# dan64/vs-deoldify

Hardware: AMD Instinct MI355X
Metric: colorized frames/sec/GPU @1080p (DeOldify stable rf=35); CIEDE2000 vs ref (higher is better)
Workload: dtype f16

## Files before the change

vsdeoldify_amd/csrc/conv_igemm.hip:

```cpp
#include "conv_common.h"

__device__ __forceinline__ int swz(int row) { return (4 - ((row >> 2) & 3)) & 3; }

template <int BM, int BN, int WM, int WN, bool PRECISE = false>
__global__ void __launch_bounds__(256, (BN > 256 ? 1 : 2)) conv_igemm_kernel(const ConvArgs p) {
    constexpr int FM = BM / WM / 16;
    constexpr int FN = BN / WN / 16;
    constexpr int A_IT = BM * 4 / 256;
    constexpr int B_IT = (BN * 4 + 255) / 256;
    constexpr int STAGE = (BM + BN) * 32;
    static_assert(BM % 64 == 0, "BM");
    __shared__ __attribute__((aligned(16))) half_t smem[2 * STAGE];

    const int tid = threadIdx.x;
    const int lane = tid & 63, wave = tid >> 6;
    const int wm = wave / WN, wn = wave % WN;
    const int lr = lane & 15, lg = lane >> 4;

    const int nwg = gridDim.x;
    int pid;
    {
        const int orig = blockIdx.x, xcd = orig & 7, q = nwg >> 3, r = nwg & 7;
        pid = (xcd < r ? xcd * (q + 1) : r * (q + 1) + (xcd - r) * q) + (orig >> 3);
    }
// ... 120 lines not shown
    const int64_t blocks128 = (int64_t)((a.M + 127) / 128) * ((a.Npad + 127) / 128);
    if (a.Npad <= 64) return a.M >= 128 * 256 ? CFG_128x64 : CFG_64x64;
    if (blocks128 >= 512) return CFG_128x128;
    const int64_t blocks64x128 = (int64_t)((a.M + 63) / 64) * ((a.Npad + 127) / 128);
    if (blocks64x128 >= 512 || a.Npad % 128 == 0) return CFG_64x128;
    return CFG_64x64;
}

bool conv_pipe_supported(const ConvArgs& a, int extra);

static int pick_pipe(const ConvArgs& a) {
    if (a.flags & HAVC_F_OUT_RGB8) return 0;
    const int extra = (a.Npad % 256 == 16) ? 1 : 0;
    if (!conv_pipe_supported(a, extra)) return 0;
    if (a.flags & HAVC_F_PS_BLUR) return extra ? 0 : 60;
    if (a.flags & HAVC_F_FUSE_RGB8) return 61;
    if (a.flags & HAVC_F_FUSE_PROJ) return (extra || a.Npad % 256) ? 0 : 60;
    if (a.Npad >= 256 && (a.Npad % 256 == 0 || extra)) {
        const int64_t blocks = (int64_t)((a.M + 255) / 256) * ((a.Npad - 16 * extra) / 256);
        if (blocks >= 160) return 60 + extra;
    }
    if (a.Npad % 128 == 0) {
        const int64_t blocks128 = (int64_t)((a.M + 127) / 128) * (a.Npad / 128);
        return blocks128 >= 200 ? 70 : 72;
    }
    return 0;
}

const char* conv_config_name(const ConvArgs& a) {
    switch (pick_pipe(a)) {
        case 60: return "pipe256x256";
        case 61: return "pipe256x272";
        case 70: return "pipe128x128";
        case 72: return "pipe64x128";
    }
    static const char* names[] = {"128x128", "128x64", "64x64", "128x272", "128x304", "128x16", "64x128"};
    return names[pick_config(a)];
}

int launch_conv(const ConvArgs& a, hipStream_t s) {
    if (a.splitk > 1) {
        int cfg = a.cfg;
        if (!conv_splitk_cfg_ok(cfg)) cfg = a.Npad % 256 == 0 ? 71 : (a.Npad % 128 == 0 ? 72 : (a.Npad <= 64 ? 92 : 72));
        if (!conv_pipe_supported(a, 0)) return (int)hipErrorInvalidValue;
        return launch_conv_pipe(a, cfg, s);
    }
    if ((a.flags & HAVC_F_FUSE_PROJ) && a.cfg != 0 && a.cfg != 60) return (int)hipErrorInvalidValue;
// ... 20 lines not shown
```

vsdeoldify_amd/csrc/conv_igemm_pipe.hip:

```cpp
#include "conv_common.h"
#include <atomic>
#include <cstdio>
#include <cstdlib>
#include <type_traits>

#include "conv_pipe_kernel.inc"

template <int EXTRA, int ABL = 0>
__global__ void __launch_bounds__(512) conv_halo_kernel(const ConvArgs p) {
    constexpr int WM = 2, WN = 4, FM = 8, NW = 8, BM = 256, BN = 256, B_IT = BN / 8 / NW, NS = 16;
    constexpr int HB = 46 * 1024, WB = (BN + 16 * EXTRA) * 128, H_IT = 6, HP = 144;
    extern __shared__ __attribute__((aligned(16))) char smem[];
    char* const Wbase = smem + 2 * HB;

    const int tid = threadIdx.x;
    const int lane = tid & 63;
    const int wave = __builtin_amdgcn_readfirstlane(tid >> 6);
    const int wm = wave / WN, wn = wave % WN;
    const int lr = lane & 15, lg = lane >> 4;

    const int nwg = gridDim.x;
    int pid;
    {
        const int orig = blockIdx.x, xcd = orig & 7, q = nwg >> 3, r = nwg & 7;
        pid = (xcd < r ? xcd * (q + 1) : r * (q + 1) + (xcd - r) * q) + (orig >> 3);
    }
    const int NT = (p.Npad - 16 * EXTRA + BN - 1) / BN;
    const int tile = pid / NT;
    const int m0 = tile * BM;
    const int n0 = (pid % NT) * BN;
    const bool has_extra = EXTRA && (n0 + BN + 16 == p.Npad);
    const int HoWo = p.Ho * p.Wo;
    const int tt = p.tiles_y * p.tiles_x;
    const int tb = tile / tt, trem = tile - tb * tt, ty = trem / p.tiles_x, tx = trem - ty * p.tiles_x;

    const __amdgpu_buffer_rsrc_t rx = __builtin_amdgcn_make_buffer_rsrc(const_cast<half_t*>(p.x), 0, p.x_bytes, 0x00020000);
    const __amdgpu_buffer_rsrc_t rw = __builtin_amdgcn_make_buffer_rsrc(const_cast<half_t*>(p.w), 0, p.w_bytes, 0x00020000);

    const int r8 = lane >> 3;
    const int c = (lane & 7) ^ ((((wave & 1) << 2) + (r8 >> 1)) & 7);
    unsigned b_voff[B_IT];
#pragma unroll
    for (int it = 0; it < B_IT; ++it) {
        const int n = n0 + (wave + it * NW) * 8 + r8;
        b_voff[it] = n < p.Npad ? (unsigned)((n * p.Kc + c) * 16) : OOB;
    }
    const unsigned x_voff = (unsigned)(((n0 + BN + (wave & 1) * 8 + r8) * p.Kc + c) * 16);
    const bool extra_wave = has_extra && wave >= 6;

    unsigned h_voff[H_IT];
#pragma unroll
    for (int it = 0; it < H_IT; ++it) {
        const int piece = wave + it * NW;
        const int sl = piece * 64 + lane;
        const int row = sl / 9, col = sl - row * 9;
        const int hy = row / 18, hx = row - hy * 18;
        const int iy = ty * 16 - 1 + hy, ix = tx * 16 - 1 + hx;
        const bool ok = piece < 46 && row < 324 && col < 8 && (unsigned)iy < (unsigned)p.Hi && (unsigned)ix < (unsigned)p.Wi;
        const int chunk = (col & 4) | ((col & 1) << 1) | ((col >> 1) & 1);
        const unsigned off = (unsigned)((((int64_t)(tb * p.Hi + iy) * p.Wi + ix) * p.x_cpitch + p.x_coff) * 2) + (unsigned)chunk * 16u;
        h_voff[it] = ok ? (off | (col == 0 ? 1u : 0u)) : OOB;
    }
    const int G = p.C8a >> 3;
    const int KT = p.Kc >> 3;
    const bool has_rem = KT > 9 * G;

    const int fsw = (lr >> 1) & 7;
    const int b_l0 = (wn * 64 + lr) * 128 + ((lg ^ fsw) << 4), b_l1 = b_l0 ^ 64;
    const int x_l0 = (BN + lr) * 128 + ((lg ^ fsw) << 4), x_l1 = x_l0 ^ 64;
    const int lp = lr < 4 ? 2 * lr : (lr < 12 ? 2 * (lr - 4) + 1 : 2 * (lr - 8));
    const int a_row = (wm * 8 * 18 + lp) * HP;
    int a_cur = a_row + (((lg & 1) << 1) | (lg >> 1)) * 16, a_nxt = a_cur + HB;
    auto tap_off = [](int t) { return ((t / 3) * 18 + (t % 3)) * HP; };
    const int rem_buf = (G & 1) * HB;
    const int a_rem0 = rem_buf + a_row + tap_off(lg), a_rem1 = rem_buf + a_row + tap_off(4 + lg), a_rem8 = rem_buf + a_row + tap_off(8);

    float4v acc[FN][FM];
    float4v accx[2];
#pragma unroll
    for (int ni = 0; ni < FN; ++ni)
#pragma unroll
        for (int mi = 0; mi < FM; ++mi) acc[ni][mi] = float4v{0.f, 0.f, 0.f, 0.f};
    accx[0] = accx[1] = float4v{0.f, 0.f, 0.f, 0.f};

    auto w_piece = [&](int q, char* wbuf, int kstage, bool live = true) {
        dma16(rw, wbuf + (wave + q * NW) * 1024, (ABL == 6 || !live) ? OOB : b_voff[q], (unsigned)kstage * 128u);
    };
    auto h_piece = [&](int it, int hoff, int group, bool rem, bool live = true) {
        const unsigned v = h_voff[it];
        const unsigned vr = (v & 1u) ? (v & ~1u) : OOB;
        const unsigned vo = (ABL == 6 || !live) ? OOB : (rem ? vr : (v & ~1u));
        dma16(rx, smem + hoff + (wave + it * NW) * 1024, vo, (unsigned)group * 128u);
    };

#pragma unroll
    for (int it = 0; it < H_IT; ++it) if (wave + it * NW < 46) h_piece(it, 0, 0, G == 0);
#pragma unroll
    for (int q = 0; q < B_IT; ++q) w_piece(q, Wbase, 0);
    if (EXTRA && extra_wave) dma16(rw, Wbase + BN * 128 + (wave & 1) * 1024, x_voff, 0);
    if (KT > 1) {
#pragma unroll
        for (int q = 0; q < B_IT; ++q) w_piece(q, Wbase + WB, 1);
        if (EXTRA && extra_wave) dma16(rw, Wbase + WB + BN * 128 + (wave & 1) * 1024, x_voff, 128u);
    }
    asm volatile("s_waitcnt vmcnt(0)" ::: "memory");
    __builtin_amdgcn_s_barrier();

    half8 bf[2][FN];
    half8 xb[2];
    half8 af[4];
#pragma unroll
    for (int ni = 0; ni < FN; ++ni) bf[0][ni] = *reinterpret_cast<const half8*>(Wbase + b_l0 + ni * 2048);
    if (EXTRA) xb[0] = *reinterpret_cast<const half8*>(Wbase + x_l0);
    {
        const int a0 = G > 0 ? a_cur : a_rem0;
        af[0] = *reinterpret_cast<const half8*>(smem + a0);
        af[1] = *reinterpret_cast<const half8*>(smem + a0 + 18 * HP);
    }
    int h_cur_off = 0;

    auto stage = [&](int kt, int group, auto t_tag, int a_next) {
        constexpr int T = decltype(t_tag)::value;
        constexpr bool DMA_ON = ABL != 1;
        const char* wcur = Wbase + (kt & 1) * WB;
        char* wnxt = Wbase + ((kt & 1) ^ 1) * WB;
        const bool more2 = kt + 2 < KT;
#pragma unroll
        for (int s = 0; s < NS; ++s) {
            const int ks = s / FM, mi = s % FM;
            if (s + 2 < NS) {
                const int s2 = s + 2, k2 = s2 / FM, m2 = s2 % FM;
                int addr;
                if (T < 9) addr = a_cur + tap_off(T) + m2 * 18 * HP + k2 * 64;
                else if (T == 9) addr = (k2 ? a_rem1 : a_rem0) + m2 * 18 * HP;
                else addr = a_rem8 + m2 * 18 * HP;
                af[s2 % 4] = *reinterpret_cast<const half8*>(smem + addr);
            }
            if (s == NS - 3) {
                asm volatile("s_waitcnt vmcnt(0) lgkmcnt(0)" ::: "memory");
                __builtin_amdgcn_s_barrier();
            }
            if (s >= NS - 2) {
                const int j = s - (NS - 2);
                af[(s + 2) % 4] = *reinterpret_cast<const half8*>(smem + a_next + j * 18 * HP);
#pragma unroll
                for (int ni = 2 * j; ni < 2 * j + 2; ++ni) bf[0][ni] = *reinterpret_cast<const half8*>(wnxt + b_l0 + ni * 2048);
                if (EXTRA && j == 1) xb[0] = *reinterpret_cast<const half8*>(wnxt + x_l0);
            }
            if (ks == 0 && mi >= FM - FN)
                bf[1][mi - (FM - FN)] = *reinterpret_cast<const half8*>(wcur + b_l1 + (mi - (FM - FN)) * 2048);
            if (EXTRA && s == 3) xb[1] = *reinterpret_cast<const half8*>(wcur + x_l1);
            if (DMA_ON) {
                if (s >= NS - 3) {
                    char* wc = const_cast<char*>(wcur);
                    if (s == NS - 3) w_piece(0, wc, kt + 2, more2);
                    if (s == NS - 2) { w_piece(1, wc, kt + 2, more2); w_piece(2, wc, kt + 2, more2); }
                    if (s == NS - 1) {
                        w_piece(3, wc, kt + 2, more2);
                        if (EXTRA) { if (extra_wave) dma16(rw, wc + BN * 128 + (wave & 1) * 1024, more2 ? x_voff : OOB, (unsigned)(kt + 2) * 128u); }
                    }
                }
                if (T < H_IT && s == 6) {
                    if (T < H_IT - 1 || wave + T * NW < 46) h_piece(T, h_cur_off ^ HB, group + 1, group + 1 >= G, group + 1 < G || has_rem);
                }
            }
            const half8 a = af[s % 4];
#pragma unroll
            for (int ni = 0; ni < FN; ++ni) {
                if (ABL == 4) asm volatile("" ::"v"(bf[ks][ni]), "v"(a));
                else acc[ni][mi] = __builtin_amdgcn_mfma_f32_16x16x32_f16(bf[ks][ni], a, acc[ni][mi], 0, 0, 0);
            }
            if (EXTRA && has_extra) {
                if (wn == (mi >> 1)) accx[mi & 1] = __builtin_amdgcn_mfma_f32_16x16x32_f16(xb[ks], a, accx[mi & 1], 0, 0, 0);
            }
            __builtin_amdgcn_sched_barrier(0);
        }
    };
    int kt = 0;
    for (int g = 0; g < G; ++g) {
        stage(kt++, g, std::integral_constant<int, 0>{}, a_cur + tap_off(1));
        stage(kt++, g, std::integral_constant<int, 1>{}, a_cur + tap_off(2));
        stage(kt++, g, std::integral_constant<int, 2>{}, a_cur + tap_off(3));
        stage(kt++, g, std::integral_constant<int, 3>{}, a_cur + tap_off(4));
        stage(kt++, g, std::integral_constant<int, 4>{}, a_cur + tap_off(5));
        stage(kt++, g, std::integral_constant<int, 5>{}, a_cur + tap_off(6));
        stage(kt++, g, std::integral_constant<int, 6>{}, a_cur + tap_off(7));
        stage(kt++, g, std::integral_constant<int, 7>{}, a_cur + tap_off(8));
        stage(kt++, g, std::integral_constant<int, 8>{}, g + 1 < G ? a_nxt : a_rem0);
        const int t = a_cur; a_cur = a_nxt; a_nxt = t;
        h_cur_off ^= HB;
    }
    if (has_rem) {
        stage(kt++, G, std::integral_constant<int, 9>{}, a_rem8);
        stage(kt++, G, std::integral_constant<int, 10>{}, a_rem8);
    }

    auto gm = [&](int local_row) -> int {
        const int y = ty * 16 + (local_row >> 4), x = tx * 16 + (local_row & 15);
        return (y < p.Ho && x < p.Wo) ? (tb * p.Ho + y) * p.Wo + x : 0x7fffffff;
    };
#define PF(mi) (mi)
#define HAVC_STAMP(i) do { } while (0)
    const int eflags = p.flags;
    constexpr bool UNIT_STEP = false;
    auto opix = [&](int m) -> int64_t { return (int64_t)m; };
#include "conv_pipe_epilogue.inc"
#undef PF
#undef HAVC_STAMP
}

template <int EXTRA, int ABL = 0>
static int launch_halo(const ConvArgs& a0, hipStream_t s) {
    ConvArgs a = a0;
    if ((a.Kc & 7) || a.x_bytes == 0 || a.x_bytes >= OOB || a.w_bytes >= OOB || a.kh != 3 || a.kw != 3 || a.stride != 1 || a.pad != 1 ||
        a.pad_w != 1 || a.dil != 1 || a.oss != 1 || a.Hi != a.Ho || a.Wi != a.Wo)
        return (int)hipErrorInvalidValue;
    const int frames = a.M / (a.Ho * a.Wo);
    a.tiles_y = (a.Ho + 15) / 16;
    a.tiles_x = (a.Wo + 15) / 16;
    const int MT = frames * a.tiles_y * a.tiles_x, NT = (a.Npad - 16 * EXTRA + 255) / 256;
    a.M = MT * 256;
    constexpr int LDS = 2 * 46 * 1024 + 2 * (256 + 16 * EXTRA) * 128;
    static_assert(LDS <= 160 * 1024, "LDS budget");
    ensure_lds_optin<conv_halo_kernel<EXTRA, ABL>>(LDS);
    hipLaunchKernelGGL((conv_halo_kernel<EXTRA, ABL>), dim3(MT * NT), dim3(512), LDS, s, a);
    return (int)hipGetLastError();
}

__global__ void splitk_reduce_kernel(const ConvArgs p) {
    const int n4 = p.Npad >> 2, HoWo = p.Ho * p.Wo;
    const int64_t total = (int64_t)p.M * n4;
    for (int64_t i = blockIdx.x * (int64_t)blockDim.x + threadIdx.x; i < total; i += (int64_t)gridDim.x * blockDim.x) {
        const int m = (int)(i / n4), n = (int)(i - (int64_t)m * n4) * 4;
        float4v acc = *reinterpret_cast<const float4v*>(p.ws + (int64_t)m * p.Npad + n);
        for (int sp = 1; sp < p.splitk; ++sp) {
            const float4v t = *reinterpret_cast<const float4v*>(p.ws + ((int64_t)sp * p.M + m) * p.Npad + n);
            acc[0] += t[0]; acc[1] += t[1]; acc[2] += t[2]; acc[3] += t[3];
        }
        epilogue_frag(p, acc, m, n, HoWo);
    }
}

// ... 18 lines not shown
    const int64_t work = (int64_t)a.M * (a.Npad >> 2);
    const int64_t gb = (work + 255) / 256;
    hipLaunchKernelGGL(splitk_reduce_kernel, dim3((unsigned)(gb > 8192 ? 8192 : gb)), dim3(256), 0, s, a);
    return (int)hipGetLastError();
}

void preload_conv_pipe() {
#define PL(WM, WN, FM, EX, ABL) ensure_lds_optin<conv_pipe_kernel<WM, WN, FM, EX, ABL>>(Geo<WM, WN, FM, EX>::LDS_BYTES)
    PL(2, 4, 8, 0, 0); PL(2, 4, 8, 1, 0); PL(2, 2, 4, 0, 0); PL(1, 4, 8, 0, 0); PL(1, 2, 4, 0, 0);
    PL(1, 4, 6, 0, 0); PL(1, 4, 4, 0, 0); PL(2, 2, 6, 0, 0); PL(1, 2, 6, 0, 0); PL(2, 4, 4, 0, 0); PL(2, 4, 6, 0, 0); PL(4, 2, 4, 0, 0);
    PL(4, 1, 4, 0, 0); PL(2, 1, 4, 0, 0);
    PL(2, 4, 8, 0, 30); PL(2, 4, 8, 1, 30); PL(2, 2, 4, 0, 30); PL(1, 4, 8, 0, 30); PL(1, 2, 4, 0, 30); PL(2, 4, 4, 0, 30); PL(4, 2, 4, 0, 30);
    PL(4, 1, 4, 0, 30); PL(2, 1, 4, 0, 30);
#undef PL
    preload_conv_pipe_ef();
    ensure_lds_optin<conv_halo_kernel<0, 0>>(2 * 46 * 1024 + 2 * 256 * 128);
    ensure_lds_optin<conv_halo_kernel<1, 0>>(2 * 46 * 1024 + 2 * 272 * 128);
    (void)hipGetLastError();
}

bool conv_splitk_cfg_ok(int cfg) {
    switch (cfg) { case 60: case 70: case 71: case 72: case 90: case 91: case 92: case 93: case 95: case 96: case 97: case 98: case 99: return true; }
    return false;
}

bool conv_pipe_supported(const ConvArgs& a, int extra) {
    return !(a.Kc & 7) && a.ktab && a.x_bytes != 0 && a.x_bytes < OOB && a.w_bytes < OOB && (!extra || a.Npad == 272);
}

int launch_conv_pipe(const ConvArgs& a, int cfg, hipStream_t s) {
    if (a.flags & HAVC_F_PRECISE) {
        switch (cfg) {
            case 60: return launch_pipe<2, 4, 8, 0, 30>(a, s);
            case 61: return launch_pipe<2, 4, 8, 1, 30>(a, s);
            case 70: return launch_pipe<2, 2, 4, 0, 30>(a, s);
            case 71: return launch_pipe<1, 4, 8, 0, 30>(a, s);
            case 72: return launch_pipe<1, 2, 4, 0, 30>(a, s);
            case 96: return launch_pipe<2, 4, 4, 0, 30>(a, s);
            case 98: return launch_pipe<4, 2, 4, 0, 30>(a, s);
            case 99: return launch_pipe<4, 1, 4, 0, 30>(a, s);
            case 92: return launch_pipe<2, 1, 4, 0, 30>(a, s);
        }
        return (int)hipErrorInvalidValue;
    }
    {
        const int r = launch_conv_pipe_ef(a, cfg, s);
        if (r != -1) return r;
        static const bool trace = getenv("HAVC_EPI_TRACE") != nullptr;
        if (trace) {
            static std::atomic<uint64_t> seen[64];
            const uint64_t key = ((uint64_t)cfg << 32) | (uint32_t)(a.flags & 0xffff) | ((uint64_t)(a.splitk > 1) << 48) | ((uint64_t)(a.oss != 1) << 49) | ((uint64_t)(!a.bias) << 50);
            for (auto& e : seen) {
                uint64_t cur = e.load();
                if (cur == key) break;
                if (cur == 0 && e.compare_exchange_strong(cur, key)) {
                    fprintf(stderr, "havc: run-time-flag conv kernel: cfg %d flags 0x%x splitk %d out_step %d bias %d (M %d, N %d, K %d)\n", cfg, a.flags & 0xffff, a.splitk, a.oss,
                            a.bias != nullptr, a.M, a.Npad, a.Kc * 8);
                    break;
                }
                if (cur == key) break;
            }
// ... 8 lines not shown
        case 103: return launch_pipe<2, 4, 8, 1, 22>(a, s);
        case 62: return launch_pipe<2, 4, 8, 0, 1>(a, s);
        case 64: return launch_pipe<2, 4, 8, 0, 4>(a, s);
        case 69: return launch_pipe<2, 4, 8, 0, 9>(a, s);
        case 73: return launch_pipe<2, 4, 8, 0, 10>(a, s);
        case 65: return launch_pipe<2, 4, 8, 0, 5>(a, s);
        case 162: return launch_pipe<2, 4, 8, 0, 40, 0>(a, s);
        case 163: return launch_pipe<2, 4, 8, 0, 40, HAVC_F_GELU>(a, s);
        case 164: return launch_pipe<2, 4, 8, 1, 40, HAVC_F_RELU_PRE>(a, s);
        case 68: return launch_pipe<2, 4, 8, 0, 12>(a, s);
        case 78: return launch_pipe<2, 4, 8, 0, 14>(a, s);
        case 66: return launch_pipe<2, 4, 8, 0, 11>(a, s);
        case 67: return launch_pipe<2, 4, 8, 0, 13>(a, s);
        case 80: return launch_halo<0>(a, s);
        case 81: return launch_halo<1>(a, s);
        case 82: return launch_halo<0, 1>(a, s);
        case 84: return launch_halo<0, 4>(a, s);
        case 85: return launch_halo<0, 5>(a, s);
        case 86: return launch_halo<0, 6>(a, s);
        case 70: return launch_pipe<2, 2, 4, 0>(a, s);
        case 71: return launch_pipe<1, 4, 8, 0>(a, s);
        case 72: return launch_pipe<1, 2, 4, 0>(a, s);
        case 90: return launch_pipe<1, 4, 6, 0>(a, s);
        case 91: return launch_pipe<1, 4, 4, 0>(a, s);
        case 93: return launch_pipe<2, 2, 6, 0>(a, s);
        case 95: return launch_pipe<1, 2, 6, 0>(a, s);
        case 96: return launch_pipe<2, 4, 4, 0>(a, s);
        case 97: return launch_pipe<2, 4, 6, 0>(a, s);
        case 98: return launch_pipe<4, 2, 4, 0>(a, s);
        case 99: return launch_pipe<4, 1, 4, 0>(a, s);
// ... 9 lines not shown
```

vsdeoldify_amd/csrc/kernels.h:

```cpp
#pragma once
#include <hip/hip_runtime.h>
#include <stdint.h>

typedef _Float16 half_t;

struct ConvArgs {
    const half_t* x;
    const half_t* w;
    const float* bias;
    const float* scale;
    const float* shift;
    const half_t* res;
    void* y;
    int x_cpitch, x_coff;
    int res_cpitch, res_coff;
    int y_cpitch, y_coff;
    int Hi, Wi, C8;
    int Ho, Wo, Co;
    int kh, kw, stride, pad, dil;
    int pad_w;
    int oss, ooy, oox;
    int Kc, Npad;
    int M;
    int flags;
// ... 20 lines not shown
inline void conv_raster(ConvArgs& a, int MT, int NT, int BN) {
    static const int on = [] { const char* e = getenv("HAVC_RASTER_GROUP"); return e ? atoi(e) : 0; }();
    a.ngroup = a.rband = 0;
    const double tile_bytes = (double)BN * a.Kc * 16.0;
    if (!on || a.splitk > 1 || NT < 4 || MT < 16 || tile_bytes * NT < 3.5e6) return;
    int ng = (int)(2.5e6 / tile_bytes);
    if (ng < 2 || ng >= NT) return;
    a.ngroup = ng;
    a.rband = (MT + 7) / 8;
}
#define HAVC_KTAB_PAD_DH 0x7fff

int launch_conv(const ConvArgs& a, hipStream_t s);
int launch_conv_pipe(const ConvArgs& a, int cfg, hipStream_t s);
int launch_conv_pipe_ef(const ConvArgs& a, int cfg, hipStream_t s);
bool conv_splitk_cfg_ok(int cfg);
const char* conv_config_name(const ConvArgs& a);

int launch_maxpool3x3s2(const half_t* x, half_t* y, int B, int Hi, int Wi, int Ho, int Wo, int C, int x_cpitch,
                        int x_coff, int y_cpitch, int y_coff, hipStream_t s);
int launch_blur_resize(const half_t* x, half_t* y, int B, int Hi, int Wi, int Ho, int Wo, int C, int x_cpitch,
                       int x_coff, int y_cpitch, int y_coff, hipStream_t s);
int launch_affine(const half_t* x, half_t* y, const float* scale, const float* shift, int relu, int64_t npix, int C,
                  int x_cpitch, int x_coff, int y_cpitch, int y_coff, hipStream_t s);
int launch_copy_ch(const half_t* x, half_t* y, int64_t npix, int C, int x_cpitch, int x_coff, int y_cpitch,
                   int y_coff, hipStream_t s);
int launch_prep_rgb8(const uint8_t* rgb, half_t* y0, int y0_cpitch, int y0_coff, half_t* y1, int y1_cpitch,
                     int y1_coff, int64_t npix, hipStream_t s, int y1_fill = 0);
int launch_subsample2(const half_t* x, half_t* y, int B, int Ho, int Wo, int Hi, int Wi, int C, int x_cpitch, int x_coff,
                      int y_cpitch, int y_coff, hipStream_t s);
// ... 84 lines not shown
int launch_mem_topk_readout(const float* sim, const float* mv, int* idx, float* wgt, float* cand_val, int* cand_idx, float* out, int B, int CV, int N,
                            int HW, int K, hipStream_t s, int64_t vpitch = 0);
int launch_mem_usage_update(const int* idx, const float* wgt, unsigned long long* acc, float* use, float* life, int from, int N, int HW, int K, hipStream_t s);
int launch_cmn_value_in(const float* img, const float* planes, float* vin, int64_t P, hipStream_t s);
int launch_vec_add(float* y, const float* x, int64_t n, hipStream_t s);
int launch_cmn_frame_in(const uint8_t* rgb, float* lab, float* img, int w, int h, int Wp, int Hp, int pad_l, int pad_t, hipStream_t s);
int launch_cmn_frame_out(const float* l_plane, const float* ab, uint8_t* rgb, int w, int h, int Wp, int Hp, int pad_l, int pad_t, hipStream_t s);
int launch_local_correlation(const float* q, const float* k, float* out, int n, int C, int H, int W, int R, int dil, float qscale, hipStream_t s);
int launch_local_softmax(float* qk, const float* q, const float* rel_w, const float* rel_b, int n, int C, int H, int W, int R, int dil, hipStream_t s);
int launch_local_agg(const float* attn, const float* v, float* agg, int n, int CV, int H, int W, int R, int dil, hipStream_t s);

int launch_range_stats(const void* p, int elem_bytes, int64_t n, unsigned* stats, hipStream_t s);

void preload_conv_pipe();
void preload_conv_pipe_ef();
void preload_conv_igemm();
void preload_elementwise();
void preload_zhang();
void preload_attention();
void preload_colorfilters();
void preload_tweaks();
void preload_ddcolor();
void preload_colormnet();
void preload_colormnet_net();
void preload_precise();

int launch_prep_rgb8_p(const uint8_t* rgb, half_t* y0, int y0_cpitch, int y0_coff, half_t* y1, int y1_cpitch, int y1_coff, int64_t npix, hipStream_t s);
int launch_maxpool3x3s2_p(const half_t* x, half_t* y, int B, int Hi, int Wi, int Ho, int Wo, int C, int x_cpitch, int x_coff, int y_cpitch, int y_coff,
                          hipStream_t s);
int launch_blur_resize_p(const half_t* x, half_t* y, int B, int Hi, int Wi, int Ho, int Wo, int C, int x_cpitch, int x_coff, int y_cpitch, int y_coff,
// ... 64 lines not shown
```

Measured before the change: 361.3.

## Enable halo-tiled 3x3 conv kernel with specialized epilogues for 272-channel RGB8-fused layers

Moves the halo conv kernel into a shared include and adds compile-time epilogue-flag specializations. The kernel loads one 18x18 spatial halo per channel group and reuses it across all nine taps, and it is now selected by default for 3x3 stride-1 convolutions with Npad 272 and fused RGB8 output. The extra 16-column weight tile is now computed with rotated fragment ordering across waves. A timestamp-instrumented variant is also added for profiling. The aim is to cut redundant activation loads and epilogue branching, at the cost of a large LDS footprint and more template instances.

New measurement: 362.9, median of 6. Within noise of the previous version (+0.4%).

```diff
diff --git a/vsdeoldify_amd/csrc/conv_halo_kernel.inc b/vsdeoldify_amd/csrc/conv_halo_kernel.inc
--- /dev/null
+++ b/vsdeoldify_amd/csrc/conv_halo_kernel.inc
@@ -0,0 +1,267 @@
+template <int EXTRA, int ABL = 0, int EF = -1>
+__global__ void __launch_bounds__(512) conv_halo_kernel(const ConvArgs p) {
+    constexpr int WM = 2, WN = 4, FM = 8, NW = 8, BM = 256, BN = 256, B_IT = BN / 8 / NW, NS = 16;
+    constexpr int HB = 46 * 1024, WB = (BN + 16 * EXTRA) * 128, H_IT = 6, HP = 144;
+    extern __shared__ __attribute__((aligned(16))) char smem[];
+    char* const Wbase = smem + 2 * HB;
+
+    uint64_t stamps[10] = {0, 0, 0, 0, 0, 0, 0, 0, 0, 0};
+#define HAVC_STAMP(i) do { if (ABL == 40) stamps[i] = __builtin_amdgcn_s_memtime(); } while (0)
+    HAVC_STAMP(0);
+    const int tid = threadIdx.x;
+    const int lane = tid & 63;
+    const int wave = __builtin_amdgcn_readfirstlane(tid >> 6);
+    const int wm = wave / WN, wn = wave % WN;
+    const int lr = lane & 15, lg = lane >> 4;
+
+    const int nwg = gridDim.x;
+    int pid;
+    {
+        const int orig = blockIdx.x, xcd = orig & 7, q = nwg >> 3, r = nwg & 7;
+        pid = (xcd < r ? xcd * (q + 1) : r * (q + 1) + (xcd - r) * q) + (orig >> 3);
+    }
+    const int NT = EXTRA ? 1 : (p.Npad + BN - 1) / BN;
+    const int tile = NT == 1 ? pid : pid / NT;
+    const int m0 = tile * BM;
+    const int n0 = (pid - tile * NT) * BN;
+    constexpr bool has_extra = EXTRA != 0;
+    const int HoWo = p.Ho * p.Wo;
+
+    const __amdgpu_buffer_rsrc_t rx = __builtin_amdgcn_make_buffer_rsrc(const_cast<half_t*>(p.x), 0, p.x_bytes, 0x00020000);
+    const __amdgpu_buffer_rsrc_t rw = __builtin_amdgcn_make_buffer_rsrc(const_cast<half_t*>(p.w), 0, p.w_bytes, 0x00020000);
+
+    const int r8 = lane >> 3;
+    const int c = (lane & 7) ^ ((((wave & 1) << 2) + (r8 >> 1)) & 7);
+    unsigned b_voff[B_IT];
+#pragma unroll
+    for (int it = 0; it < B_IT; ++it) {
+        const int n = n0 + (wave + it * NW) * 8 + r8;
+        b_voff[it] = n < p.Npad ? (unsigned)((n * p.Kc + c) * 16) : OOB;
+    }
+    const bool extra_wave = has_extra && wave >= 6;
+    const int KT = p.Kc >> 3;
+    const unsigned wrow = (unsigned)p.Kc * 16u;
+    const unsigned x_soff = (unsigned)(BN - (wave & ~1) * 8) * wrow;
+    auto w_piece = [&](int q, char* wbuf, int kstage, bool live = true) {
+        const bool dead = ABL == 6 || !live;
+        if (EXTRA) dma16(rw, wbuf + (wave + q * NW) * 1024, dead ? OOB : b_voff[0], (unsigned)kstage * 128u + (unsigned)(q * NW * 8) * wrow);
+        else dma16(rw, wbuf + (wave + q * NW) * 1024, dead ? OOB : b_voff[q], (unsigned)kstage * 128u);
+    };
+    auto x_piece = [&](char* wbuf, int kstage, bool live = true) {
+        if (extra_wave) dma16(rw, wbuf + BN * 128 + (wave & 1) * 1024, live ? b_voff[0] : OOB, (unsigned)kstage * 128u + x_soff);
+    };
+    HAVC_STAMP(8);
+#pragma unroll
+    for (int q = 0; q < B_IT; ++q) w_piece(q, Wbase, 0);
+    if (EXTRA) x_piece(Wbase, 0);
+    if (KT > 1) {
+#pragma unroll
+        for (int q = 0; q < B_IT; ++q) w_piece(q, Wbase + WB, 1);
+        if (EXTRA) x_piece(Wbase + WB, 1);
+    }
+    const int tt = p.tiles_y * p.tiles_x;
+    const int tb = tile / tt, trem = tile - tb * tt, ty = trem / p.tiles_x, tx = trem - ty * p.tiles_x;
+
+    unsigned h_voff[H_IT];
+#pragma unroll
+    for (int it = 0; it < H_IT; ++it) {
+        const int piece = wave + it * NW;
+        const int sl = piece * 64 + lane;
+        const int row = sl / 9, col = sl - row * 9;
+        const int hy = row / 18, hx = row - hy * 18;
+        const int iy = ty * 16 - 1 + hy, ix = tx * 16 - 1 + hx;
+        const bool ok = piece < 46 && row < 324 && col < 8 && (unsigned)iy < (unsigned)p.Hi && (unsigned)ix < (unsigned)p.Wi;
+        const int chunk = (col & 4) | ((col & 1) << 1) | ((col >> 1) & 1);
+        const unsigned off = (unsigned)((((int64_t)(tb * p.Hi + iy) * p.Wi + ix) * p.x_cpitch + p.x_coff) * 2) + (unsigned)chunk * 16u;
+        h_voff[it] = ok ? (off | (col == 0 ? 1u : 0u)) : OOB;
+    }
+    const int G = p.C8a >> 3;
+    const bool has_rem = KT > 9 * G;
+
+    const int fsw = (lr >> 1) & 7;
+    const int b_l0 = (wn * 64 + lr) * 128 + ((lg ^ fsw) << 4), b_l1 = b_l0 ^ 64;
+    const int x_d = (BN - wn * 64) * 128;
+    const int lp = lr < 4 ? 2 * lr : (lr < 12 ? 2 * (lr - 4) + 1 : 2 * (lr - 8));
+    const int a_row = (wm * 8 * 18 + lp) * HP;
+    int ro[FM];
+#pragma unroll
+    for (int mi = 0; mi < FM; ++mi) ro[mi] = (EXTRA ? ((mi + 2 * wn) & (FM - 1)) : mi) * (18 * HP);
+#define PF(mi) (EXTRA ? (((mi) + 2 * wn) & (FM - 1)) : (mi))
+    const int a_main = a_row + (((lg & 1) << 1) | (lg >> 1)) * 16;
+    auto sofs = [](int v) -> int { asm volatile("" : "+s"(v)); return v; };
+    constexpr auto tap_off = [](int t) constexpr { return ((t / 3) * 18 + (t % 3)) * HP; };
+    const int rem_buf = (G & 1) * HB;
+    const int a_rem0 = a_row + tap_off(lg);
+
+    float4v acc[FN][FM];
+    float4v accx[2];
+#pragma unroll
+    for (int ni = 0; ni < FN; ++ni)
+#pragma unroll
+        for (int mi = 0; mi < FM; ++mi) acc[ni][mi] = float4v{0.f, 0.f, 0.f, 0.f};
+    accx[0] = accx[1] = float4v{0.f, 0.f, 0.f, 0.f};
+
+    auto h_piece = [&](int it, int hoff, int group, bool rem, bool live = true) {
+        const unsigned v = h_voff[it];
+        const unsigned vr = (v & 1u) ? (v & ~1u) : OOB;
+        const unsigned vo = (ABL == 6 || !live) ? OOB : (rem ? vr : (v & ~1u));
+        dma16(rx, smem + hoff + (wave + it * NW) * 1024, vo, (unsigned)group * 128u);
+    };
+
+#pragma unroll
+    for (int it = 0; it < H_IT; ++it) if (wave + it * NW < 46) h_piece(it, 0, 0, G == 0);
+    HAVC_STAMP(9);
+    asm volatile("s_waitcnt vmcnt(0)" ::: "memory");
+    __builtin_amdgcn_s_barrier();
+    HAVC_STAMP(1);
+
+    half8 bf[2][FN];
+    half8 xb[2];
+    half8 af[4];
+#pragma unroll
+    for (int ni = 0; ni < FN; ++ni) bf[0][ni] = *reinterpret_cast<const half8*>(Wbase + b_l0 + ni * 2048);
+    if (EXTRA) xb[0] = *reinterpret_cast<const half8*>(Wbase + b_l0 + sofs(x_d));
+    {
+        const int a0 = G > 0 ? a_main : a_rem0;
+        af[0] = *reinterpret_cast<const half8*>(smem + a0 + sofs(ro[0]));
+        af[1] = *reinterpret_cast<const half8*>(smem + a0 + sofs(ro[1]));
+    }
+    int h_cur_off = 0;
+
+    auto stage = [&](int kt, int group, auto t_tag, int nv, int ns, auto ni_tag, int a_r1 = 0, int a_r8 = 0) {
+        constexpr int T = decltype(t_tag)::value, NI = decltype(ni_tag)::value;
+        constexpr bool DMA_ON = ABL != 1;
+        const char* wcur = Wbase + (kt & 1) * WB;
+        const int wc_o = (kt & 1) * WB, wn_o = WB - wc_o;
+        const bool more2 = kt + 2 < KT;
+#pragma unroll
+        for (int s = 0; s < NS; ++s) {
+            const int ks = s / FM, mi = s % FM;
+            if (s + 2 < NS) {
+                const int s2 = s + 2, k2 = s2 / FM, m2 = s2 % FM;
+                int addr;
+                if (T < 9) addr = a_main + sofs(h_cur_off + ro[m2]) + (tap_off(T) + k2 * 64);
+                else if (T == 9) addr = (k2 ? a_r1 : a_rem0) + sofs(rem_buf + ro[m2]);
+                else addr = a_r8 + sofs(rem_buf + ro[m2]) + tap_off(8);
+                af[s2 % 4] = *reinterpret_cast<const half8*>(smem + addr);
+            }
+            if (s == NS - 3) {
+                asm volatile("s_waitcnt vmcnt(0) lgkmcnt(0)" ::: "memory");
+                __builtin_amdgcn_s_barrier();
+            }
+            if (s >= NS - 2) {
+                const int j = s - (NS - 2);
+                af[(s + 2) % 4] = *reinterpret_cast<const half8*>(smem + (nv + sofs(ns + ro[j]) + NI));
+#pragma unroll
+                for (int ni = 2 * j; ni < 2 * j + 2; ++ni) bf[0][ni] = *reinterpret_cast<const half8*>(Wbase + (b_l0 + sofs(wn_o)) + ni * 2048);
+                if (EXTRA && j == 1) xb[0] = *reinterpret_cast<const half8*>(Wbase + (b_l0 + sofs(wn_o + x_d)));
+            }
+            if (ks == 0 && mi >= FM - FN)
+                bf[1][mi - (FM - FN)] = *reinterpret_cast<const half8*>(Wbase + (b_l1 + sofs(wc_o)) + (mi - (FM - FN)) * 2048);
+            if (EXTRA && s == 3) xb[1] = *reinterpret_cast<const half8*>(Wbase + (b_l1 + sofs(wc_o + x_d)));
+            if (DMA_ON) {
+                if (s >= NS - 3) {
+                    char* wc = const_cast<char*>(wcur);
+                    if (s == NS - 3) w_piece(0, wc, kt + 2, more2);
+                    if (s == NS - 2) { w_piece(1, wc, kt + 2, more2); w_piece(2, wc, kt + 2, more2); }
+                    if (s == NS - 1) {
+                        w_piece(3, wc, kt + 2, more2);
+                        if (EXTRA) x_piece(wc, kt + 2, more2);
+                    }
+                }
+                if (T < H_IT && s == 6) {
+                    if (T < H_IT - 1 || wave + T * NW < 46) h_piece(T, h_cur_off ^ HB, group + 1, group + 1 >= G, group + 1 < G || has_rem);
+                }
+            }
+            const half8 a = af[s % 4];
+#pragma unroll
+            for (int ni = 0; ni < FN; ++ni) {
+                if (ABL == 4) asm volatile("" ::"v"(bf[ks][ni]), "v"(a));
+                else acc[ni][mi] = __builtin_amdgcn_mfma_f32_16x16x32_f16(bf[ks][ni], a, acc[ni][mi], 0, 0, 0);
+            }
+            if (EXTRA && mi < 2)
+                accx[mi] = __builtin_amdgcn_mfma_f32_16x16x32_f16(xb[ks], a, accx[mi], 0, 0, 0);
+            __builtin_amdgcn_sched_barrier(0);
+        }
+    };
+    int kt = 0;
+#define HAVC_TAP(T) std::integral_constant<int, T>{}
+#define HAVC_NI(T) std::integral_constant<int, tap_off(T)>{}
+    for (int g = 0; g < G; ++g) {
+        stage(kt++, g, HAVC_TAP(0), a_main, h_cur_off, HAVC_NI(1));
+        stage(kt++, g, HAVC_TAP(1), a_main, h_cur_off, HAVC_NI(2));
+        stage(kt++, g, HAVC_TAP(2), a_main, h_cur_off, HAVC_NI(3));
+        stage(kt++, g, HAVC_TAP(3), a_main, h_cur_off, HAVC_NI(4));
+        stage(kt++, g, HAVC_TAP(4), a_main, h_cur_off, HAVC_NI(5));
+        stage(kt++, g, HAVC_TAP(5), a_main, h_cur_off, HAVC_NI(6));
+        stage(kt++, g, HAVC_TAP(6), a_main, h_cur_off, HAVC_NI(7));
+        stage(kt++, g, HAVC_TAP(7), a_main, h_cur_off, HAVC_NI(8));
+        stage(kt++, g, HAVC_TAP(8), g + 1 < G ? a_main : a_rem0, h_cur_off ^ HB, HAVC_NI(0));
+        h_cur_off ^= HB;
+    }
+    if (has_rem) {
+        int t2 = tid;
+        asm volatile("" : "+v"(t2));
+        const int lr2 = t2 & 15, lg2 = (t2 >> 4) & 3;
+        const int lp2 = lr2 < 4 ? 2 * lr2 : (lr2 < 12 ? 2 * (lr2 - 4) + 1 : 2 * (lr2 - 8));
+        const int a_row2 = (wm * 8 * 18 + lp2) * HP, a_r1 = a_row2 + tap_off(4 + lg2);
+        stage(kt++, G, HAVC_TAP(9), a_row2, rem_buf, HAVC_NI(8), a_r1, a_row2);
+        stage(kt++, G, HAVC_TAP(10), a_row2, rem_buf, HAVC_NI(8), a_r1, a_row2);
+    }
+#undef HAVC_TAP
+#undef HAVC_NI
+    HAVC_STAMP(2);
+
+    int tid_e = tid;
+    asm volatile("" : "+v"(tid_e));
+    auto gm = [&](int local_row) -> int {
+        const int y = ty * 16 + (local_row >> 4), x = tx * 16 + (local_row & 15);
+        return (y < p.Ho && x < p.Wo) ? (tb * p.Ho + y) * p.Wo + x : 0x7fffffff;
+    };
+    {
+    const int tid = tid_e, lane = tid & 63, lr = lane & 15, lg = lane >> 4;
+    const int lp = lr < 4 ? 2 * lr : (lr < 12 ? 2 * (lr - 4) + 1 : 2 * (lr - 8));
+    const int eflags = EF >= 0 ? (EF | (p.flags & ~HAVC_EPI_MASK)) : p.flags;
+    constexpr bool UNIT_STEP = EF >= 0;
+    auto opix = [&](int m) -> int64_t { return (int64_t)m; };
+#include "conv_pipe_epilogue.inc"
+    }
+#undef PF
+    if (ABL == 40) {
+        HAVC_STAMP(5);
+        asm volatile("s_waitcnt vmcnt(0)" ::: "memory");
+        HAVC_STAMP(6);
+        if (tid == 0) {
+            unsigned hwid;
+            asm volatile("s_getreg_b32 %0, hwreg(HW_REG_HW_ID)" : "=s"(hwid));
+            stamps[7] = hwid;
+            uint64_t* d = reinterpret_cast<uint64_t*>(reinterpret_cast<half_t*>(p.y) + (int64_t)gm(0) * p.y_cpitch + p.y_coff + n0);
+#pragma unroll
+            for (int i = 0; i < 10; ++i) d[i] = stamps[i];
+        }
+    }
+#undef HAVC_STAMP
+}
+
+static bool conv_halo_supported(const ConvArgs& a, int extra) {
+    const int rem = a.C8 - a.C8a;
+    return !(a.Kc & 7) && a.x_bytes != 0 && a.x_bytes < OOB && a.w_bytes < OOB && a.kh == 3 && a.kw == 3 && a.stride == 1 && a.pad == 1 && a.pad_w == 1 &&
+           a.dil == 1 && a.oss == 1 && a.Hi == a.Ho && a.Wi == a.Wo && a.C8a > 0 && (a.C8a & 7) == 0 && (rem == 0 || rem == 1) && a.Kc == 9 * a.C8a + 16 * rem &&
+           !(a.flags & HAVC_F_PRECISE) && a.splitk <= 1 && (!extra || a.Npad == 272);
+}
+
+template <int EXTRA, int ABL = 0, int EF = -1>
+static int launch_halo(const ConvArgs& a0, hipStream_t s) {
+    ConvArgs a = a0;
+    if (!conv_halo_supported(a, EXTRA) || (EF >= 0 && (a.flags & HAVC_EPI_MASK) != EF)) return (int)hipErrorInvalidValue;
+    const int frames = a.M / (a.Ho * a.Wo);
+    a.tiles_y = (a.Ho + 15) / 16;
+    a.tiles_x = (a.Wo + 15) / 16;
+    const int MT = frames * a.tiles_y * a.tiles_x, NT = (a.Npad - 16 * EXTRA + 255) / 256;
+    a.M = MT * 256;
+    constexpr int LDS = 2 * 46 * 1024 + 2 * (256 + 16 * EXTRA) * 128;
+    static_assert(LDS <= 160 * 1024, "LDS budget");
+    ensure_lds_optin<conv_halo_kernel<EXTRA, ABL, EF>>(LDS);
+    hipLaunchKernelGGL((conv_halo_kernel<EXTRA, ABL, EF>), dim3(MT * NT), dim3(512), LDS, s, a);
+    return (int)hipGetLastError();
+}
diff --git a/vsdeoldify_amd/csrc/conv_igemm.hip b/vsdeoldify_amd/csrc/conv_igemm.hip
--- a/vsdeoldify_amd/csrc/conv_igemm.hip
+++ b/vsdeoldify_amd/csrc/conv_igemm.hip
@@ -158,6 +158,11 @@
     const int extra = (a.Npad % 256 == 16) ? 1 : 0;
     if (!conv_pipe_supported(a, extra)) return 0;
     if (a.flags & HAVC_F_PS_BLUR) return extra ? 0 : 60;
+    if (a.Npad == 272 && (a.flags & HAVC_F_FUSE_RGB8) && conv_halo_selectable(a, extra)) {
+        static const bool halo_on = [] { const char* e = getenv("HAVC_HALO"); return !e || atoi(e) != 0; }();
+        const int64_t tiles = (int64_t)(a.M / (a.Ho * a.Wo)) * ((a.Ho + 15) / 16) * ((a.Wo + 15) / 16);
+        if (halo_on && tiles >= 2 * 256 && tiles <= (a.M + 255) / 256) return 80 + extra;
+    }
     if (a.flags & HAVC_F_FUSE_RGB8) return 61;
     if (a.flags & HAVC_F_FUSE_PROJ) return (extra || a.Npad % 256) ? 0 : 60;
     if (a.Npad >= 256 && (a.Npad % 256 == 0 || extra)) {
@@ -175,6 +180,8 @@
     switch (pick_pipe(a)) {
         case 60: return "pipe256x256";
         case 61: return "pipe256x272";
+        case 80: return "halo256x256";
+        case 81: return "halo256x272";
         case 70: return "pipe128x128";
         case 72: return "pipe64x128";
     }
diff --git a/vsdeoldify_amd/csrc/conv_igemm_halo_ef.hip b/vsdeoldify_amd/csrc/conv_igemm_halo_ef.hip
--- /dev/null
+++ b/vsdeoldify_amd/csrc/conv_igemm_halo_ef.hip
@@ -0,0 +1,41 @@
+#include "conv_common.h"
+#include <atomic>
+#include <cstdlib>
+#include <type_traits>
+
+#include "conv_pipe_kernel.inc"
+#include "conv_halo_kernel.inc"
+
+namespace {
+constexpr int RELU = HAVC_F_RELU_PRE, RES = HAVC_F_RESIDUAL;
+}
+
+#define HAVC_HALO_EF_ALL(X) X(1, RELU) X(1, RELU | RES | HAVC_F_FUSE_RGB8) X(0, RELU)
+
+bool conv_halo_selectable(const ConvArgs& a, int extra) {
+    if (!conv_halo_supported(a, extra)) return false;
+    const int ef = a.flags & HAVC_EPI_MASK;
+#define X(EX, EF) if (extra == EX && ef == (EF)) return true;
+    HAVC_HALO_EF_ALL(X)
+#undef X
+    return false;
+}
+
+int launch_conv_halo_ef(const ConvArgs& a, int cfg, hipStream_t s) {
+    static const bool on = [] { const char* e = getenv("HAVC_EPI_SPECIAL"); return !e || atoi(e) != 0; }();
+    if (!on || (cfg != 80 && cfg != 81)) return -1;
+    const int ef = a.flags & HAVC_EPI_MASK;
+#define X(EX, EF) if (cfg == 80 + EX && ef == (EF)) return launch_halo<EX, 0, (EF)>(a, s);
+    HAVC_HALO_EF_ALL(X)
+#undef X
+    return -1;
+}
+
+int launch_conv_halo_stamped(const ConvArgs& a, hipStream_t s) { return launch_halo<1, 40, RELU>(a, s); }
+
+void preload_conv_halo_ef() {
+#define X(EX, EF) ensure_lds_optin<conv_halo_kernel<EX, 0, (EF)>>(2 * 46 * 1024 + 2 * (256 + 16 * EX) * 128);
+    HAVC_HALO_EF_ALL(X)
+#undef X
+    (void)hipGetLastError();
+}
diff --git a/vsdeoldify_amd/csrc/conv_igemm_pipe.hip b/vsdeoldify_amd/csrc/conv_igemm_pipe.hip
--- a/vsdeoldify_amd/csrc/conv_igemm_pipe.hip
+++ b/vsdeoldify_amd/csrc/conv_igemm_pipe.hip
@@ -6,226 +6,7 @@
 
 #include "conv_pipe_kernel.inc"
 
-template <int EXTRA, int ABL = 0>
-__global__ void __launch_bounds__(512) conv_halo_kernel(const ConvArgs p) {
-    constexpr int WM = 2, WN = 4, FM = 8, NW = 8, BM = 256, BN = 256, B_IT = BN / 8 / NW, NS = 16;
-    constexpr int HB = 46 * 1024, WB = (BN + 16 * EXTRA) * 128, H_IT = 6, HP = 144;
-    extern __shared__ __attribute__((aligned(16))) char smem[];
-    char* const Wbase = smem + 2 * HB;
-
-    const int tid = threadIdx.x;
-    const int lane = tid & 63;
-    const int wave = __builtin_amdgcn_readfirstlane(tid >> 6);
-    const int wm = wave / WN, wn = wave % WN;
-    const int lr = lane & 15, lg = lane >> 4;
-
-    const int nwg = gridDim.x;
-    int pid;
-    {
-        const int orig = blockIdx.x, xcd = orig & 7, q = nwg >> 3, r = nwg & 7;
-        pid = (xcd < r ? xcd * (q + 1) : r * (q + 1) + (xcd - r) * q) + (orig >> 3);
-    }
-    const int NT = (p.Npad - 16 * EXTRA + BN - 1) / BN;
-    const int tile = pid / NT;
-    const int m0 = tile * BM;
-    const int n0 = (pid % NT) * BN;
-    const bool has_extra = EXTRA && (n0 + BN + 16 == p.Npad);
-    const int HoWo = p.Ho * p.Wo;
-    const int tt = p.tiles_y * p.tiles_x;
-    const int tb = tile / tt, trem = tile - tb * tt, ty = trem / p.tiles_x, tx = trem - ty * p.tiles_x;
-
-    const __amdgpu_buffer_rsrc_t rx = __builtin_amdgcn_make_buffer_rsrc(const_cast<half_t*>(p.x), 0, p.x_bytes, 0x00020000);
-    const __amdgpu_buffer_rsrc_t rw = __builtin_amdgcn_make_buffer_rsrc(const_cast<half_t*>(p.w), 0, p.w_bytes, 0x00020000);
-
-    const int r8 = lane >> 3;
-    const int c = (lane & 7) ^ ((((wave & 1) << 2) + (r8 >> 1)) & 7);
-    unsigned b_voff[B_IT];
-#pragma unroll
-    for (int it = 0; it < B_IT; ++it) {
-        const int n = n0 + (wave + it * NW) * 8 + r8;
-        b_voff[it] = n < p.Npad ? (unsigned)((n * p.Kc + c) * 16) : OOB;
-    }
-    const unsigned x_voff = (unsigned)(((n0 + BN + (wave & 1) * 8 + r8) * p.Kc + c) * 16);
-    const bool extra_wave = has_extra && wave >= 6;
-
-    unsigned h_voff[H_IT];
-#pragma unroll
-    for (int it = 0; it < H_IT; ++it) {
-        const int piece = wave + it * NW;
-        const int sl = piece * 64 + lane;
-        const int row = sl / 9, col = sl - row * 9;
-        const int hy = row / 18, hx = row - hy * 18;
-        const int iy = ty * 16 - 1 + hy, ix = tx * 16 - 1 + hx;
-        const bool ok = piece < 46 && row < 324 && col < 8 && (unsigned)iy < (unsigned)p.Hi && (unsigned)ix < (unsigned)p.Wi;
-        const int chunk = (col & 4) | ((col & 1) << 1) | ((col >> 1) & 1);
-        const unsigned off = (unsigned)((((int64_t)(tb * p.Hi + iy) * p.Wi + ix) * p.x_cpitch + p.x_coff) * 2) + (unsigned)chunk * 16u;
-        h_voff[it] = ok ? (off | (col == 0 ? 1u : 0u)) : OOB;
-    }
-    const int G = p.C8a >> 3;
-    const int KT = p.Kc >> 3;
-    const bool has_rem = KT > 9 * G;
-
-    const int fsw = (lr >> 1) & 7;
-    const int b_l0 = (wn * 64 + lr) * 128 + ((lg ^ fsw) << 4), b_l1 = b_l0 ^ 64;
-    const int x_l0 = (BN + lr) * 128 + ((lg ^ fsw) << 4), x_l1 = x_l0 ^ 64;
-    const int lp = lr < 4 ? 2 * lr : (lr < 12 ? 2 * (lr - 4) + 1 : 2 * (lr - 8));
-    const int a_row = (wm * 8 * 18 + lp) * HP;
-    int a_cur = a_row + (((lg & 1) << 1) | (lg >> 1)) * 16, a_nxt = a_cur + HB;
-    auto tap_off = [](int t) { return ((t / 3) * 18 + (t % 3)) * HP; };
-    const int rem_buf = (G & 1) * HB;
-    const int a_rem0 = rem_buf + a_row + tap_off(lg), a_rem1 = rem_buf + a_row + tap_off(4 + lg), a_rem8 = rem_buf + a_row + tap_off(8);
-
-    float4v acc[FN][FM];
-    float4v accx[2];
-#pragma unroll
-    for (int ni = 0; ni < FN; ++ni)
-#pragma unroll
-        for (int mi = 0; mi < FM; ++mi) acc[ni][mi] = float4v{0.f, 0.f, 0.f, 0.f};
-    accx[0] = accx[1] = float4v{0.f, 0.f, 0.f, 0.f};
-
-    auto w_piece = [&](int q, char* wbuf, int kstage, bool live = true) {
-        dma16(rw, wbuf + (wave + q * NW) * 1024, (ABL == 6 || !live) ? OOB : b_voff[q], (unsigned)kstage * 128u);
-    };
-    auto h_piece = [&](int it, int hoff, int group, bool rem, bool live = true) {
-        const unsigned v = h_voff[it];
-        const unsigned vr = (v & 1u) ? (v & ~1u) : OOB;
-        const unsigned vo = (ABL == 6 || !live) ? OOB : (rem ? vr : (v & ~1u));
-        dma16(rx, smem + hoff + (wave + it * NW) * 1024, vo, (unsigned)group * 128u);
-    };
-
-#pragma unroll
-    for (int it = 0; it < H_IT; ++it) if (wave + it * NW < 46) h_piece(it, 0, 0, G == 0);
-#pragma unroll
-    for (int q = 0; q < B_IT; ++q) w_piece(q, Wbase, 0);
-    if (EXTRA && extra_wave) dma16(rw, Wbase + BN * 128 + (wave & 1) * 1024, x_voff, 0);
-    if (KT > 1) {
-#pragma unroll
-        for (int q = 0; q < B_IT; ++q) w_piece(q, Wbase + WB, 1);
-        if (EXTRA && extra_wave) dma16(rw, Wbase + WB + BN * 128 + (wave & 1) * 1024, x_voff, 128u);
-    }
-    asm volatile("s_waitcnt vmcnt(0)" ::: "memory");
-    __builtin_amdgcn_s_barrier();
-
-    half8 bf[2][FN];
-    half8 xb[2];
-    half8 af[4];
-#pragma unroll
-    for (int ni = 0; ni < FN; ++ni) bf[0][ni] = *reinterpret_cast<const half8*>(Wbase + b_l0 + ni * 2048);
-    if (EXTRA) xb[0] = *reinterpret_cast<const half8*>(Wbase + x_l0);
-    {
-        const int a0 = G > 0 ? a_cur : a_rem0;
-        af[0] = *reinterpret_cast<const half8*>(smem + a0);
-        af[1] = *reinterpret_cast<const half8*>(smem + a0 + 18 * HP);
-    }
-    int h_cur_off = 0;
-
-    auto stage = [&](int kt, int group, auto t_tag, int a_next) {
-        constexpr int T = decltype(t_tag)::value;
-        constexpr bool DMA_ON = ABL != 1;
-        const char* wcur = Wbase + (kt & 1) * WB;
-        char* wnxt = Wbase + ((kt & 1) ^ 1) * WB;
-        const bool more2 = kt + 2 < KT;
-#pragma unroll
-        for (int s = 0; s < NS; ++s) {
-            const int ks = s / FM, mi = s % FM;
-            if (s + 2 < NS) {
-                const int s2 = s + 2, k2 = s2 / FM, m2 = s2 % FM;
-                int addr;
-                if (T < 9) addr = a_cur + tap_off(T) + m2 * 18 * HP + k2 * 64;
-                else if (T == 9) addr = (k2 ? a_rem1 : a_rem0) + m2 * 18 * HP;
-                else addr = a_rem8 + m2 * 18 * HP;
-                af[s2 % 4] = *reinterpret_cast<const half8*>(smem + addr);
-            }
-            if (s == NS - 3) {
-                asm volatile("s_waitcnt vmcnt(0) lgkmcnt(0)" ::: "memory");
-                __builtin_amdgcn_s_barrier();
-            }
-            if (s >= NS - 2) {
-                const int j = s - (NS - 2);
-                af[(s + 2) % 4] = *reinterpret_cast<const half8*>(smem + a_next + j * 18 * HP);
-#pragma unroll
-                for (int ni = 2 * j; ni < 2 * j + 2; ++ni) bf[0][ni] = *reinterpret_cast<const half8*>(wnxt + b_l0 + ni * 2048);
-                if (EXTRA && j == 1) xb[0] = *reinterpret_cast<const half8*>(wnxt + x_l0);
-            }
-            if (ks == 0 && mi >= FM - FN)
-                bf[1][mi - (FM - FN)] = *reinterpret_cast<const half8*>(wcur + b_l1 + (mi - (FM - FN)) * 2048);
-            if (EXTRA && s == 3) xb[1] = *reinterpret_cast<const half8*>(wcur + x_l1);
-            if (DMA_ON) {
-                if (s >= NS - 3) {
-                    char* wc = const_cast<char*>(wcur);
-                    if (s == NS - 3) w_piece(0, wc, kt + 2, more2);
-                    if (s == NS - 2) { w_piece(1, wc, kt + 2, more2); w_piece(2, wc, kt + 2, more2); }
-                    if (s == NS - 1) {
-                        w_piece(3, wc, kt + 2, more2);
-                        if (EXTRA) { if (extra_wave) dma16(rw, wc + BN * 128 + (wave & 1) * 1024, more2 ? x_voff : OOB, (unsigned)(kt + 2) * 128u); }
-                    }
-                }
-                if (T < H_IT && s == 6) {
-                    if (T < H_IT - 1 || wave + T * NW < 46) h_piece(T, h_cur_off ^ HB, group + 1, group + 1 >= G, group + 1 < G || has_rem);
-                }
-            }
-            const half8 a = af[s % 4];
-#pragma unroll
-            for (int ni = 0; ni < FN; ++ni) {
-                if (ABL == 4) asm volatile("" ::"v"(bf[ks][ni]), "v"(a));
-                else acc[ni][mi] = __builtin_amdgcn_mfma_f32_16x16x32_f16(bf[ks][ni], a, acc[ni][mi], 0, 0, 0);
-            }
-            if (EXTRA && has_extra) {
-                if (wn == (mi >> 1)) accx[mi & 1] = __builtin_amdgcn_mfma_f32_16x16x32_f16(xb[ks], a, accx[mi & 1], 0, 0, 0);
-            }
-            __builtin_amdgcn_sched_barrier(0);
-        }
-    };
-    int kt = 0;
-    for (int g = 0; g < G; ++g) {
-        stage(kt++, g, std::integral_constant<int, 0>{}, a_cur + tap_off(1));
-        stage(kt++, g, std::integral_constant<int, 1>{}, a_cur + tap_off(2));
-        stage(kt++, g, std::integral_constant<int, 2>{}, a_cur + tap_off(3));
-        stage(kt++, g, std::integral_constant<int, 3>{}, a_cur + tap_off(4));
-        stage(kt++, g, std::integral_constant<int, 4>{}, a_cur + tap_off(5));
-        stage(kt++, g, std::integral_constant<int, 5>{}, a_cur + tap_off(6));
-        stage(kt++, g, std::integral_constant<int, 6>{}, a_cur + tap_off(7));
-        stage(kt++, g, std::integral_constant<int, 7>{}, a_cur + tap_off(8));
-        stage(kt++, g, std::integral_constant<int, 8>{}, g + 1 < G ? a_nxt : a_rem0);
-        const int t = a_cur; a_cur = a_nxt; a_nxt = t;
-        h_cur_off ^= HB;
-    }
-    if (has_rem) {
-        stage(kt++, G, std::integral_constant<int, 9>{}, a_rem8);
-        stage(kt++, G, std::integral_constant<int, 10>{}, a_rem8);
-    }
-
-    auto gm = [&](int local_row) -> int {
-        const int y = ty * 16 + (local_row >> 4), x = tx * 16 + (local_row & 15);
-        return (y < p.Ho && x < p.Wo) ? (tb * p.Ho + y) * p.Wo + x : 0x7fffffff;
-    };
-#define PF(mi) (mi)
-#define HAVC_STAMP(i) do { } while (0)
-    const int eflags = p.flags;
-    constexpr bool UNIT_STEP = false;
-    auto opix = [&](int m) -> int64_t { return (int64_t)m; };
-#include "conv_pipe_epilogue.inc"
-#undef PF
-#undef HAVC_STAMP
-}
-
-template <int EXTRA, int ABL = 0>
-static int launch_halo(const ConvArgs& a0, hipStream_t s) {
-    ConvArgs a = a0;
-    if ((a.Kc & 7) || a.x_bytes == 0 || a.x_bytes >= OOB || a.w_bytes >= OOB || a.kh != 3 || a.kw != 3 || a.stride != 1 || a.pad != 1 ||
-        a.pad_w != 1 || a.dil != 1 || a.oss != 1 || a.Hi != a.Ho || a.Wi != a.Wo)
-        return (int)hipErrorInvalidValue;
-    const int frames = a.M / (a.Ho * a.Wo);
-    a.tiles_y = (a.Ho + 15) / 16;
-    a.tiles_x = (a.Wo + 15) / 16;
-    const int MT = frames * a.tiles_y * a.tiles_x, NT = (a.Npad - 16 * EXTRA + 255) / 256;
-    a.M = MT * 256;
-    constexpr int LDS = 2 * 46 * 1024 + 2 * (256 + 16 * EXTRA) * 128;
-    static_assert(LDS <= 160 * 1024, "LDS budget");
-    ensure_lds_optin<conv_halo_kernel<EXTRA, ABL>>(LDS);
-    hipLaunchKernelGGL((conv_halo_kernel<EXTRA, ABL>), dim3(MT * NT), dim3(512), LDS, s, a);
-    return (int)hipGetLastError();
-}
+#include "conv_halo_kernel.inc"
 
 __global__ void splitk_reduce_kernel(const ConvArgs p) {
     const int n4 = p.Npad >> 2, HoWo = p.Ho * p.Wo;
@@ -274,6 +55,7 @@
     PL(4, 1, 4, 0, 30); PL(2, 1, 4, 0, 30);
 #undef PL
     preload_conv_pipe_ef();
+    preload_conv_halo_ef();
     ensure_lds_optin<conv_halo_kernel<0, 0>>(2 * 46 * 1024 + 2 * 256 * 128);
     ensure_lds_optin<conv_halo_kernel<1, 0>>(2 * 46 * 1024 + 2 * 272 * 128);
     (void)hipGetLastError();
@@ -304,7 +86,8 @@
         return (int)hipErrorInvalidValue;
     }
     {
-        const int r = launch_conv_pipe_ef(a, cfg, s);
+        int r = launch_conv_pipe_ef(a, cfg, s);
+        if (r == -1) r = launch_conv_halo_ef(a, cfg, s);
         if (r != -1) return r;
         static const bool trace = getenv("HAVC_EPI_TRACE") != nullptr;
         if (trace) {
@@ -343,6 +126,7 @@
         case 67: return launch_pipe<2, 4, 8, 0, 13>(a, s);
         case 80: return launch_halo<0>(a, s);
         case 81: return launch_halo<1>(a, s);
+        case 181: return launch_conv_halo_stamped(a, s);
         case 82: return launch_halo<0, 1>(a, s);
         case 84: return launch_halo<0, 4>(a, s);
         case 85: return launch_halo<0, 5>(a, s);
diff --git a/vsdeoldify_amd/csrc/kernels.h b/vsdeoldify_amd/csrc/kernels.h
--- a/vsdeoldify_amd/csrc/kernels.h
+++ b/vsdeoldify_amd/csrc/kernels.h
@@ -58,6 +58,9 @@
 int launch_conv(const ConvArgs& a, hipStream_t s);
 int launch_conv_pipe(const ConvArgs& a, int cfg, hipStream_t s);
 int launch_conv_pipe_ef(const ConvArgs& a, int cfg, hipStream_t s);
+int launch_conv_halo_ef(const ConvArgs& a, int cfg, hipStream_t s);
+int launch_conv_halo_stamped(const ConvArgs& a, hipStream_t s);
+bool conv_halo_selectable(const ConvArgs& a, int extra);
 bool conv_splitk_cfg_ok(int cfg);
 const char* conv_config_name(const ConvArgs& a);
 
@@ -172,6 +175,7 @@
 
 void preload_conv_pipe();
 void preload_conv_pipe_ef();
+void preload_conv_halo_ef();
 void preload_conv_igemm();
 void preload_elementwise();
 void preload_zhang();
```
